# MikeIvanichev/norma

Measured on AMD Instinct MI355X. Metric: audio-sec/wall-sec (xRT) distil-large-v3 fp16 b32, higher is better.
Workload: dtype f16

## Files before the change

### norma_amd/csrc/k_attn_enc.hip

```cpp
#include "nh_kernels.h"

#ifndef ENC_ATTN_KERNEL
#define ENC_ATTN_KERNEL enc_attn_kernel
#define ENC_ATTN_LAUNCH launch_enc_attention
#endif
#define KT 64
#define QW 32
#ifndef ENC_ATTN_WAVES
#define ENC_ATTN_WAVES 8
#endif
#define QB (QW * ENC_ATTN_WAVES)
#define NTHR (64 * ENC_ATTN_WAVES)
#define NSLOT (NTHR >= 512 ? 1 : 512 / NTHR)
#define TILE_B 8192

__device__ __forceinline__ int swap23(int x) { return (x & ~12) | ((x & 4) << 1) | ((x & 8) >> 1); }

#ifndef ENC_ATTN_MINWAVES
#ifdef ENC_ATTN_PIPE
#define ENC_ATTN_MINWAVES 2
#else
#define ENC_ATTN_MINWAVES 4
#endif
#endif
__global__ __launch_bounds__(NTHR, (NTHR <= 512 ? ENC_ATTN_MINWAVES : 1)) void ENC_ATTN_KERNEL(const half_t *__restrict__ q, const half_t *__restrict__ k,
                                                         long ld, const half_t *__restrict__ vt,
                                                         half_t *__restrict__ out, long ldo, int S, int H) {
    __shared__ __attribute__((aligned(16))) char smem[2 * 2 * TILE_B];
    const int tid = threadIdx.x, lane = tid & 63, w = tid >> 6;
    const int r = lane & 31, hh = lane >> 5;
    const int b = blockIdx.z, h = blockIdx.y;
    const int q0 = blockIdx.x * QB + w * QW;
    const int nT = (S + KT - 1) / KT;

    half8 qf[4];
    {
        int qrow = q0 + r; if (qrow >= S) qrow = S - 1;
        const half_t *qp = q + ((long)b * S + qrow) * ld + h * NH_DH + 8 * hh;
#pragma unroll
        for (int ks = 0; ks < 4; ks++) qf[ks] = *reinterpret_cast<const half8 *>(qp + 16 * ks);
    }
    const half_t *kg[NSLOT]; const half_t *vg[NSLOT];
    int krow_off[NSLOT];
#pragma unroll
    for (int i = 0; i < NSLOT; i++) {
        int row = (tid >> 3) + (NTHR / 8) * i;
        int c = (tid & 7) ^ ((row >> 1) & 7);
        krow_off[i] = swap23(row);
        kg[i] = k + (long)b * S * ld + h * NH_DH + c * 8;
        vg[i] = vt + ((long)(b * H + h) * NH_DH + row) * NH_SP + c * 8;
    }
    u32x4 rk[NSLOT], rv[NSLOT];
    const bool stager = NTHR <= 512 || tid < 512;
    auto load_k = [&](int t) {
        if (!stager) return;
#pragma unroll
        for (int i = 0; i < NSLOT; i++) {
            int key = t * KT + krow_off[i]; if (key >= S) key = S - 1;
            rk[i] = *reinterpret_cast<const u32x4 *>(kg[i] + (long)key * ld);
        }
    };
    auto load_v = [&](int t) {
        if (!stager) return;
#pragma unroll
        for (int i = 0; i < NSLOT; i++) rv[i] = *reinterpret_cast<const u32x4 *>(vg[i] + t * KT);
    };
    auto store_k = [&](int buf) {
        if (!stager) return;
        u32x4 *lk = reinterpret_cast<u32x4 *>(smem + buf * 2 * TILE_B);
#pragma unroll
        for (int i = 0; i < NSLOT; i++) lk[tid + NTHR * i] = rk[i];
    };
    auto store_v = [&](int buf) {
        if (!stager) return;
        u32x4 *lv = reinterpret_cast<u32x4 *>(smem + buf * 2 * TILE_B + TILE_B);
#pragma unroll
        for (int i = 0; i < NSLOT; i++) lv[tid + NTHR * i] = rv[i];
    };
    auto load_tile = [&](int t) { load_k(t); load_v(t); };
    auto store_tile = [&](int buf) { store_k(buf); store_v(buf); };
    load_tile(0);
    store_tile(0);
#ifdef ENC_ATTN_PIPE
    if (nT > 1) { load_k(1); store_k(1); }
#endif
    __syncthreads();

    const int g = (r >> 1) & 7;
    const int offK0 = r * 128 + ((hh ^ g) << 4);
    const int offV0 = r * 128 + ((hh ^ g) << 4);

    f32x16 o0, o1;
#pragma unroll
    for (int i = 0; i < 16; i++) { o0[i] = 0.f; o1[i] = 0.f; }
    const f32x16 zero = {0.f, 0.f, 0.f, 0.f, 0.f, 0.f, 0.f, 0.f, 0.f, 0.f, 0.f, 0.f, 0.f, 0.f, 0.f, 0.f};
    const half_t one_h = hh == 0 ? (half_t)1.0f : (half_t)0.0f;
    const half8 kx = {one_h, one_h, (half_t)0.f, (half_t)0.f, (half_t)0.f, (half_t)0.f, (half_t)0.f, (half_t)0.f};
    half8 qx = {(half_t)0.f, (half_t)0.f, (half_t)0.f, (half_t)0.f, (half_t)0.f, (half_t)0.f, (half_t)0.f, (half_t)0.f};
    float m_ref = 0.f, l_run = 0.f;
    const float REBASE = 8.0f;

    f32x16 s0, s1;
    auto qk_phase = [&](const char *tk, f32x16 &s0, f32x16 &s1) {
        {
            half8 k0 = *reinterpret_cast<const half8 *>(tk + offK0);
            half8 k1 = *reinterpret_cast<const half8 *>(tk + 4096 + offK0);
            s0 = __builtin_amdgcn_mfma_f32_32x32x16_f16(k0, qf[0], zero, 0, 0, 0);
            s1 = __builtin_amdgcn_mfma_f32_32x32x16_f16(k1, qf[0], zero, 0, 0, 0);
        }
#pragma unroll
        for (int ks = 1; ks < 4; ks++) {
            half8 k0 = *reinterpret_cast<const half8 *>(tk + (offK0 ^ (ks << 5)));
            half8 k1 = *reinterpret_cast<const half8 *>(tk + 4096 + (offK0 ^ (ks << 5)));
            s0 = __builtin_amdgcn_mfma_f32_32x32x16_f16(k0, qf[ks], s0, 0, 0, 0);
            s1 = __builtin_amdgcn_mfma_f32_32x32x16_f16(k1, qf[ks], s1, 0, 0, 0);
        }
        s0 = __builtin_amdgcn_mfma_f32_32x32x16_f16(kx, qx, s0, 0, 0, 0);
        s1 = __builtin_amdgcn_mfma_f32_32x32x16_f16(kx, qx, s1, 0, 0, 0);
    };
    auto sm_head = [&](int t) {
        if (t * KT + KT > S) {
#pragma unroll
            for (int i = 0; i < 16; i++) {
                int rho = (i & 3) + 8 * (i >> 2) + 4 * hh;
                int key0 = t * KT + swap23(rho), key1 = t * KT + 32 + swap23(rho);
                if (key0 >= S) s0[i] = -INFINITY;
                if (key1 >= S) s1[i] = -INFINITY;
            }
        }
        float mx = fmaxf(fmaxf(s0[0], s0[1]), s0[2]);
#pragma unroll
        for (int i = 3; i < 15; i += 2) mx = fmaxf(fmaxf(mx, s0[i]), s0[i + 1]);
        mx = fmaxf(fmaxf(mx, s0[15]), s1[0]);
#pragma unroll
        for (int i = 1; i < 15; i += 2) mx = fmaxf(fmaxf(mx, s1[i]), s1[i + 1]);
        mx = fmaxf(mx, s1[15]);
        mx = fmaxf(mx, __shfl_xor(mx, 32));
        const bool reb = (t == 0) || (mx > REBASE);
        if (__builtin_amdgcn_ballot_w64(reb) != 0) {
            const float dlt = reb ? mx : 0.f;
            const float alpha = __builtin_amdgcn_exp2f(-dlt);
#pragma unroll
            for (int i = 0; i < 16; i++) { o0[i] *= alpha; o1[i] *= alpha; s0[i] -= dlt; s1[i] -= dlt; }
            l_run *= alpha;
            m_ref += dlt;
            const float nm = fminf(fmaxf(-m_ref, -60000.f), 60000.f);
            const half_t hi = (half_t)nm;
            const half_t lo = (half_t)(nm - (float)hi);
            qx[0] = hh == 0 ? hi : (half_t)0.f;
            qx[1] = hh == 0 ? lo : (half_t)0.f;
        }
    };
    auto sm_body = [&](const char *tv) {
        float ps = 0.f;
#pragma unroll
        for (int i = 0; i < 16; i++) {
            s0[i] = __builtin_amdgcn_exp2f(s0[i]); s1[i] = __builtin_amdgcn_exp2f(s1[i]);
            ps += s0[i]; ps += s1[i];
        }
        l_run += ps;
        half8 p00, p01, p10, p11;
#pragma unroll
        for (int j = 0; j < 8; j++) {
            p00[j] = (half_t)s0[j]; p01[j] = (half_t)s0[8 + j];
            p10[j] = (half_t)s1[j]; p11[j] = (half_t)s1[8 + j];
        }
        {
            half8 v;
            v = *reinterpret_cast<const half8 *>(tv + (offV0 ^ (0 << 4)));          o0 = __builtin_amdgcn_mfma_f32_32x32x16_f16(v, p00, o0, 0, 0, 0);
            v = *reinterpret_cast<const half8 *>(tv + 4096 + (offV0 ^ (0 << 4)));   o1 = __builtin_amdgcn_mfma_f32_32x32x16_f16(v, p00, o1, 0, 0, 0);
            v = *reinterpret_cast<const half8 *>(tv + (offV0 ^ (2 << 4)));          o0 = __builtin_amdgcn_mfma_f32_32x32x16_f16(v, p01, o0, 0, 0, 0);
            v = *reinterpret_cast<const half8 *>(tv + 4096 + (offV0 ^ (2 << 4)));   o1 = __builtin_amdgcn_mfma_f32_32x32x16_f16(v, p01, o1, 0, 0, 0);
            v = *reinterpret_cast<const half8 *>(tv + (offV0 ^ (4 << 4)));          o0 = __builtin_amdgcn_mfma_f32_32x32x16_f16(v, p10, o0, 0, 0, 0);
            v = *reinterpret_cast<const half8 *>(tv + 4096 + (offV0 ^ (4 << 4)));   o1 = __builtin_amdgcn_mfma_f32_32x32x16_f16(v, p10, o1, 0, 0, 0);
            v = *reinterpret_cast<const half8 *>(tv + (offV0 ^ (6 << 4)));          o0 = __builtin_amdgcn_mfma_f32_32x32x16_f16(v, p11, o0, 0, 0, 0);
            v = *reinterpret_cast<const half8 *>(tv + 4096 + (offV0 ^ (6 << 4)));   o1 = __builtin_amdgcn_mfma_f32_32x32x16_f16(v, p11, o1, 0, 0, 0);
        }
    };
#ifndef ENC_ATTN_PIPE
    int cur = 0;
    for (int t = 0; t < nT; t++) {
        const bool more = (t + 1 < nT);
        if (more) load_tile(t + 1);
        qk_phase(smem + cur * 2 * TILE_B, s0, s1);
        sm_head(t);
        sm_body(smem + cur * 2 * TILE_B + TILE_B);
        if (more) store_tile(cur ^ 1);
        __syncthreads();
        cur ^= 1;
    }
#else
    f32x16 n0, n1;
    qk_phase(smem, s0, s1);
    for (int t = 0; t < nT; t++) {
        if (t + 2 < nT) load_k(t + 2);
        if (t + 1 < nT) load_v(t + 1);
        sm_head(t);
        qk_phase(smem + ((t + 1) & 1) * 2 * TILE_B, n0, n1);
        sm_body(smem + (t & 1) * 2 * TILE_B + TILE_B);
#pragma unroll
        for (int i = 0; i < 18; i++) {
            __builtin_amdgcn_sched_group_barrier(0x008, 1, 0);
            __builtin_amdgcn_sched_group_barrier(0x002, ENC_ATTN_PIPE, 0);
        }
        if (t + 2 < nT) store_k(t & 1);
        if (t + 1 < nT) store_v((t + 1) & 1);
        __syncthreads();
        s0 = n0; s1 = n1;
    }
#endif
    const float l_tot = l_run + __shfl_xor(l_run, 32);
    const float inv = 1.0f / l_tot;
    const int qrow = q0 + r;
    if (qrow < S) {
        half_t *op = out + ((long)b * S + qrow) * ldo + h * NH_DH + 4 * hh;
#pragma unroll
        for (int gq = 0; gq < 4; gq++) {
            half4 a = {(half_t)(o0[4 * gq] * inv), (half_t)(o0[4 * gq + 1] * inv), (half_t)(o0[4 * gq + 2] * inv),
                       (half_t)(o0[4 * gq + 3] * inv)};
            half4 c = {(half_t)(o1[4 * gq] * inv), (half_t)(o1[4 * gq + 1] * inv), (half_t)(o1[4 * gq + 2] * inv),
                       (half_t)(o1[4 * gq + 3] * inv)};
            *reinterpret_cast<half4 *>(op + 8 * gq) = a;
            *reinterpret_cast<half4 *>(op + 32 + 8 * gq) = c;
        }
    }
}

void ENC_ATTN_LAUNCH(const half_t *q, const half_t *k, long ld, const half_t *vt, half_t *out, long ldo,
                          int B, int S, int H, hipStream_t st) {
    dim3 grid((S + QB - 1) / QB, H, B);
    hipLaunchKernelGGL(ENC_ATTN_KERNEL, grid, dim3(NTHR), 0, st, q, k, ld, vt, out, ldo, S, H);
}
```

### norma_amd/csrc/k_gemm.hip

```cpp
#include <stdlib.h>

#include <atomic>

#include "nh_kernels.h"

#define BM 128
#define BN 128
#define BK 64
#define TILE_BYTES (BM * BK * 2)

__device__ __forceinline__ float gelu_tanh_f(float v) { return gelu_tanh_fast(v); }

__device__ __forceinline__ const half_t *a_row_ptr(const GemmParams &p, int m) {
    if (m >= p.M) m = p.M - 1;
    int b = nh_div(m, p.a_rpb, p.a_magic), r = m - b * p.a_rpb;
    return p.A + (long)b * p.a_bstride + (long)r * p.lda;
}

typedef __attribute__((address_space(3))) void lds_void;
typedef const __attribute__((address_space(1))) void gbl_void;

template <bool SWAP>
__device__ __forceinline__ void gemm_mainloop(const GemmParams &p, char *smem, int m0, int n0,
                                              f32x4 (&acc)[4][4]) {
    const int tid = threadIdx.x, lane = tid & 63, w = tid >> 6;
    const int wm = w >> 1, wn = w & 1;
    const int cq = tid & 7;
    const half_t *ag[4], *wg[4];
#pragma unroll
    for (int i = 0; i < 4; i++) {
        int row = (tid >> 3) + 32 * i;
        int c = cq ^ ((row >> 1) & 7);
        ag[i] = a_row_ptr(p, m0 + row) + c * 8;
        int n = n0 + row;
        wg[i] = p.W + (long)n * p.K + c * 8;
    }
    const int nt = p.K / BK;
    const int fr = lane & 15, fq = lane >> 4;
    int offA[4], offB[4];
#pragma unroll
    for (int j = 0; j < 4; j++) {
        int rowA = wm * 64 + 16 * j + fr;
        int rowB = wn * 64 + 16 * j + fr;
        offA[j] = rowA * 128 + ((fq ^ ((rowA >> 1) & 7)) << 4);
        offB[j] = rowB * 128 + ((fq ^ ((rowB >> 1) & 7)) << 4);
    }
    const int wbase = __builtin_amdgcn_readfirstlane(w) * 1024;
    auto stage = [&](int buf, int t) {
        char *la = smem + buf * 2 * TILE_BYTES + wbase, *lb = la + TILE_BYTES;
#pragma unroll
        for (int i = 0; i < 4; i++) {
            __builtin_amdgcn_global_load_lds((gbl_void *)(ag[i] + (long)t * BK), (lds_void *)(la + 4096 * i), 16, 0, 0);
            __builtin_amdgcn_global_load_lds((gbl_void *)(wg[i] + (long)t * BK), (lds_void *)(lb + 4096 * i), 16, 0, 0);
        }
    };
    stage(0, 0);
    asm volatile("s_waitcnt vmcnt(0)" ::: "memory");
    __syncthreads();
    int cur = 0;
    for (int t = 0; t < nt; t++) {
        const bool more = (t + 1 < nt);
        if (more) stage(cur ^ 1, t + 1);
        const char *ta = smem + cur * 2 * TILE_BYTES, *tb = ta + TILE_BYTES;
#pragma unroll
        for (int ks = 0; ks < 2; ks++) {
            half8 fa[4], fb[4];
#pragma unroll
            for (int j = 0; j < 4; j++) {
                fa[j] = *reinterpret_cast<const half8 *>(ta + (offA[j] ^ (ks << 6)));
                fb[j] = *reinterpret_cast<const half8 *>(tb + (offB[j] ^ (ks << 6)));
            }
#pragma unroll
            for (int i = 0; i < 4; i++)
#pragma unroll
                for (int j = 0; j < 4; j++) {
                    if (SWAP)
                        acc[i][j] = __builtin_amdgcn_mfma_f32_16x16x32_f16(fb[i], fa[j], acc[i][j], 0, 0, 0);
                    else
                        acc[i][j] = __builtin_amdgcn_mfma_f32_16x16x32_f16(fa[j], fb[i], acc[i][j], 0, 0, 0);
                }
        }
        asm volatile("s_waitcnt vmcnt(0)" ::: "memory");
        __syncthreads();
        cur ^= 1;
    }
}

__device__ __forceinline__ long out_row(const GemmParams &p, int m) {
    int b = nh_div(m, p.o_rpb, p.o_magic), r = m - b * p.o_rpb;
    return (long)b * p.o_bstride + r + p.o_off;
}

__global__ __launch_bounds__(256, 2) void gemm_f16_kernel(GemmParams p) {
    __shared__ __attribute__((aligned(16))) char smem[4 * TILE_BYTES];
    const int ntn = p.N / BN, ntm = (p.M + BM - 1) / BM;
    const int nwg = ntn * ntm;
    int bid = blockIdx.x;
    {
        int xcd = bid & 7, q = nwg >> 3, r = nwg & 7;
        bid = (xcd < r ? xcd * (q + 1) : r * (q + 1) + (xcd - r) * q) + (bid >> 3);
    }
    const int tm = bid / ntn, tn = bid - tm * ntn;
    const int m0 = tm * BM, n0 = tn * BN;
    const int lane = threadIdx.x & 63, w = threadIdx.x >> 6;
    const int wm = w >> 1, wn = w & 1;
    const int fr = lane & 15, fq = lane >> 4;

    f32x4 acc[4][4];
#pragma unroll
    for (int i = 0; i < 4; i++)
#pragma unroll
        for (int j = 0; j < 4; j++) acc[i][j] = (f32x4){0.f, 0.f, 0.f, 0.f};

    const int seg = (p.epi == EPI_F16 || p.epi == EPI_GELU_F16) ? n0 / p.seg_n : 0;
    const bool vt = (p.epi == EPI_F16 && seg == p.vt_seg);
    if (vt) gemm_mainloop<false>(p, smem, m0, n0, acc);
    else gemm_mainloop<true>(p, smem, m0, n0, acc);

    if (vt) {
        half_t *dst = reinterpret_cast<half_t *>(seg == 0 ? p.out[0] : seg == 1 ? p.out[1] : p.out[2]);
#pragma unroll
        for (int i = 0; i < 4; i++) {
            int n = n0 + wn * 64 + 16 * i + fr;
            float bv = p.bias ? p.bias[n] : 0.f;
            int nl = n - seg * p.seg_n, h = nl >> 6, dh = nl & 63;
#pragma unroll
            for (int j = 0; j < 4; j++) {
                int m = m0 + wm * 64 + 16 * j + 4 * fq;
                if (m >= p.M) continue;
                int b = nh_div(m, p.S, p.s_magic), s = m - b * p.S;
                half_t *row = dst + ((long)(b * p.H + h) * NH_DH + dh) * NH_SP;
                if (s + 3 < p.S && m + 3 < p.M) {
                    half4 v = {(half_t)(acc[i][j][0] + bv), (half_t)(acc[i][j][1] + bv),
                               (half_t)(acc[i][j][2] + bv), (half_t)(acc[i][j][3] + bv)};
                    *reinterpret_cast<half4 *>(row + s) = v;
                } else {
                    for (int r = 0; r < 4; r++) {
                        int mm = m + r;
                        if (mm >= p.M) break;
                        int bb = nh_div(mm, p.S, p.s_magic), ss = mm - bb * p.S;
                        dst[((long)(bb * p.H + h) * NH_DH + dh) * NH_SP + ss] = (half_t)(acc[i][j][r] + bv);
                    }
                }
            }
        }
        return;
    }
    half_t *obase = reinterpret_cast<half_t *>(seg == 0 ? p.out[0] : seg == 1 ? p.out[1] : p.out[2]);
#pragma unroll
    for (int i = 0; i < 4; i++) {
        const int n = n0 + wn * 64 + 16 * i + 4 * fq;
        f32x4 bv = {0.f, 0.f, 0.f, 0.f};
        if (p.bias) bv = *reinterpret_cast<const f32x4 *>(p.bias + n);
#pragma unroll
        for (int j = 0; j < 4; j++) {
            const int m = m0 + wm * 64 + 16 * j + fr;
            if (m >= p.M) continue;
            f32x4 v = acc[i][j] + bv;
            if (p.epi == EPI_F16 || p.epi == EPI_GELU_F16) {
                if (p.epi == EPI_F16 && seg == 0 && p.seg0_scale != 0.f) v *= p.seg0_scale;
                if (p.epi == EPI_GELU_F16) {
                    v[0] = gelu_tanh_f(v[0]); v[1] = gelu_tanh_f(v[1]);
                    v[2] = gelu_tanh_f(v[2]); v[3] = gelu_tanh_f(v[3]);
                }
                const int nl = n - seg * p.seg_n;
                half_t *dst = p.head_major ? obase + (((long)nh_div(m, p.S, p.s_magic) * p.H + (nl >> 6)) * p.S + (m - nh_div(m, p.S, p.s_magic) * p.S)) * NH_DH + (nl & 63)
                                           : obase + out_row(p, m) * p.ldo + nl;
                half4 hv = {(half_t)v[0], (half_t)v[1], (half_t)v[2], (half_t)v[3]};
                *reinterpret_cast<half4 *>(dst) = hv;
            } else if (p.epi == EPI_RESID_F32) {
                float *dst = reinterpret_cast<float *>(p.out[0]) + (long)m * p.ldo + n;
                f32x4 x = *reinterpret_cast<const f32x4 *>(dst);
                *reinterpret_cast<f32x4 *>(dst) = x + v;
            } else {
                int s = m - nh_div(m, p.S, p.s_magic) * p.S;
                f32x4 pe = *reinterpret_cast<const f32x4 *>(p.pos + (long)s * p.N + n);
                f32x4 o = {gelu_tanh_f(v[0]) + pe[0], gelu_tanh_f(v[1]) + pe[1], gelu_tanh_f(v[2]) + pe[2],
                           gelu_tanh_f(v[3]) + pe[3]};
                *reinterpret_cast<f32x4 *>(reinterpret_cast<float *>(p.out[0]) + (long)m * p.ldo + n) = o;
            }
        }
    }
}

#define G2_BM 256
#define G2_BN 256
#ifndef G2_GM
#define G2_GM 4
#endif
#define PP_BUF 65536
#define PP_HT 16384
#define PP_RING (2 * PP_BUF)
#define PP_EPI_PITCH 136
#define PP_EPI_WAVE (16 * PP_EPI_PITCH)

struct PPSource { unsigned ag[2][2], wg[2][2]; };

__device__ __forceinline__ PPSource pp_source(const GemmParams &p, int m0, int n0) {
    int tid = threadIdx.x;
    asm volatile("" : "+v"(tid));
    const int lrow = tid >> 3;
    const int csrc = ((tid & 7) ^ ((lrow >> 1) & 7)) * 8;
    PPSource sg;
#pragma unroll
    for (int h = 0; h < 2; h++)
#pragma unroll
        for (int i = 0; i < 2; i++) {
            sg.ag[h][i] = (unsigned)(a_row_ptr(p, m0 + i * 128 + h * 64 + lrow) - p.A) + csrc;
            const int l = lrow + 64 * i;
            sg.wg[h][i] = (unsigned)(n0 + (l >> 5) * 64 + h * 32 + (l & 31)) * (unsigned)p.K + csrc;
        }
    return sg;
}

__device__ __forceinline__ void pp_stage(const GemmParams &p, char *wbase, const PPSource &sg, int t, int which) {
    const int h = (which >> 1) & 1;
    const bool isB = which == 1 || which == 2;
    char *dst = wbase + (t & 1) * PP_BUF + (isB ? 2 * PP_HT : 0) + h * PP_HT;
    const unsigned ko = (unsigned)t * 64u;
    if (isB) {
        __builtin_amdgcn_global_load_lds((gbl_void *)(p.W + (size_t)(sg.wg[h][0] + ko)), (lds_void *)dst, 16, 0, 0);
        __builtin_amdgcn_global_load_lds((gbl_void *)(p.W + (size_t)(sg.wg[h][1] + ko)), (lds_void *)(dst + 8192), 16, 0, 0);
    } else {
        __builtin_amdgcn_global_load_lds((gbl_void *)(p.A + (size_t)(sg.ag[h][0] + ko)), (lds_void *)dst, 16, 0, 0);
        __builtin_amdgcn_global_load_lds((gbl_void *)(p.A + (size_t)(sg.ag[h][1] + ko)), (lds_void *)(dst + 8192), 16, 0, 0);
    }
}

__device__ __forceinline__ void pp_prologue(const GemmParams &p, char *wbase, const PPSource &sg) {
    pp_stage(p, wbase, sg, 0, 0); pp_stage(p, wbase, sg, 0, 1); pp_stage(p, wbase, sg, 0, 2); pp_stage(p, wbase, sg, 0, 3);
    pp_stage(p, wbase, sg, 1, 0); pp_stage(p, wbase, sg, 1, 1);
}

template <bool SWAP>
__device__ __forceinline__ void pp_main(const GemmParams &p, char *smem, char *wbase, const PPSource &sg, f32x4 (&acc)[8][4]) {
    const int lane = threadIdx.x & 63, w = threadIdx.x >> 6;
    const int wr = w >> 2, wc = w & 3;
    const int fr = lane & 15, fq = lane >> 4;
    const int nt = p.K >> 6;
    const int offA0 = (wr * 64 + fr) * 128 + ((fq ^ (fr >> 1)) << 4);
    const int offB0 = (wc * 32 + fr) * 128 + ((fq ^ (fr >> 1)) << 4);
    const char *const pa[2] = {smem + offA0, smem + (offA0 ^ 64)};
    const char *const pb[2] = {smem + offB0, smem + (offB0 ^ 64)};
    half8 fa[4][2], fb[4][2];

#define PP_PHASE(Q, BUF, WAIT, DO_ISSUE, ST)                                                                             \
    {                                                                                                                    \
        constexpr int tb_ = (BUF) * PP_BUF;                                                                              \
        if ((Q) == 0) {                                                                                                  \
            _Pragma("unroll") for (int j = 0; j < 2; j++) _Pragma("unroll") for (int ks = 0; ks < 2; ks++)             \
                fb[j][ks] = *reinterpret_cast<const half8 *>(pb[ks] + (tb_ + 2 * PP_HT + 2048 * j));                    \
            __builtin_amdgcn_sched_barrier(0);                                                                           \
            _Pragma("unroll") for (int i = 0; i < 4; i++) _Pragma("unroll") for (int ks = 0; ks < 2; ks++)             \
                fa[i][ks] = *reinterpret_cast<const half8 *>(pa[ks] + (tb_ + 2048 * i));                               \
        } else if ((Q) == 1) {                                                                                           \
            _Pragma("unroll") for (int j = 0; j < 2; j++) _Pragma("unroll") for (int ks = 0; ks < 2; ks++)             \
                fb[2 + j][ks] = *reinterpret_cast<const half8 *>(pb[ks] + (tb_ + 3 * PP_HT + 2048 * j));                \
        } else if ((Q) == 2) {                                                                                           \
            _Pragma("unroll") for (int i = 0; i < 4; i++) _Pragma("unroll") for (int ks = 0; ks < 2; ks++)             \
                fa[i][ks] = *reinterpret_cast<const half8 *>(pa[ks] + (tb_ + PP_HT + 2048 * i));                       \
        }                                                                                                                \
        __builtin_amdgcn_sched_barrier(0);                                                                               \
        if (DO_ISSUE) pp_stage(p, wbase, sg, (ST), (Q) == 2 ? 0 : (Q) == 3 ? 1 : (Q) == 0 ? 2 : 3);                     \
        if ((WAIT) == 8) asm volatile("s_waitcnt vmcnt(8)" ::: "memory");                                                \
        else if ((WAIT) == 4) asm volatile("s_waitcnt vmcnt(4)" ::: "memory");                                           \
        else if ((WAIT) == 2) asm volatile("s_waitcnt vmcnt(2)" ::: "memory");                                           \
        else if ((WAIT) == 0) asm volatile("s_waitcnt vmcnt(0)" ::: "memory");                                           \
        __builtin_amdgcn_s_barrier();                                                                                    \
        asm volatile("s_waitcnt lgkmcnt(0)" ::: "memory");                                                               \
        __builtin_amdgcn_sched_barrier(0);                                                                               \
        __builtin_amdgcn_s_setprio(1);                                                                                   \
        {                                                                                                                \
            constexpr int ib_ = ((Q) >= 2) ? 4 : 0, jb_ = ((Q) == 1 || (Q) == 2) ? 2 : 0;                                \
            _Pragma("unroll") for (int ks = 0; ks < 2; ks++) _Pragma("unroll") for (int i = 0; i < 4; i++)             \
                _Pragma("unroll") for (int j = 0; j < 2; j++) {                                                         \
                    if (SWAP) acc[ib_ + i][jb_ + j] = __builtin_amdgcn_mfma_f32_16x16x32_f16(fb[jb_ + j][ks], fa[i][ks], acc[ib_ + i][jb_ + j], 0, 0, 0); \
                    else acc[ib_ + i][jb_ + j] = __builtin_amdgcn_mfma_f32_16x16x32_f16(fa[i][ks], fb[jb_ + j][ks], acc[ib_ + i][jb_ + j], 0, 0, 0);      \
                }                                                                                                        \
        }                                                                                                                \
        __builtin_amdgcn_s_setprio(0);                                                                                   \
        __builtin_amdgcn_sched_barrier(0);                                                                               \
        __builtin_amdgcn_s_barrier();                                                                                    \
    }

    asm volatile("s_waitcnt vmcnt(0)" ::: "memory");
    __builtin_amdgcn_s_barrier();
    if (wr == 1) __builtin_amdgcn_s_barrier();
    int t = 0;
    for (; t + 4 <= nt; t += 2) {
        PP_PHASE(0, 0, 8, true, t + 1)
        PP_PHASE(1, 0, 8, true, t + 1)
        PP_PHASE(2, 0, -1, true, t + 2)
        PP_PHASE(3, 0, 8, true, t + 2)
        PP_PHASE(0, 1, 8, true, t + 2)
        PP_PHASE(1, 1, 8, true, t + 2)
        PP_PHASE(2, 1, -1, true, t + 3)
        PP_PHASE(3, 1, 8, true, t + 3)
    }
    PP_PHASE(0, 0, 8, true, t + 1)
    PP_PHASE(1, 0, 8, true, t + 1)
    PP_PHASE(2, 0, -1, false, 0)
    PP_PHASE(3, 0, 4, false, 0)
    PP_PHASE(0, 1, 2, false, 0)
    PP_PHASE(1, 1, 0, false, 0)
    PP_PHASE(2, 1, -1, false, 0)
    PP_PHASE(3, 1, -1, false, 0)
    if (wr == 0) __builtin_amdgcn_s_barrier();
#undef PP_PHASE
}

__device__ __forceinline__ void pp_tile(int vb, int ntn, int ntm, int &tm, int &tn) {
    const int nwg = ntn * ntm;
    const int xcd = vb & 7, q = nwg >> 3, r = nwg & 7;
    const int bid = (xcd < r ? xcd * (q + 1) : r * (q + 1) + (xcd - r) * q) + (vb >> 3);
    const int per_group = G2_GM * ntn;
    const int g = bid / per_group, rr = bid - g * per_group;
    const int gm = min(G2_GM, ntm - g * G2_GM);
    tn = rr / gm; tm = g * G2_GM + (rr - tn * gm);
}

template <int EPI>
__global__ __launch_bounds__(512) void gemm256_f16_kernel(GemmParams p) {
    __shared__ __attribute__((aligned(16))) char smem[PP_RING + 8 * PP_EPI_WAVE];
    const int ntn = p.N / G2_BN, ntm = (p.M + G2_BM - 1) / G2_BM, nwg = ntn * ntm;
    const int lane = threadIdx.x & 63, w = threadIdx.x >> 6;
    const int wm = w >> 2, wn = w & 3;
    const int fr = lane & 15, fq = lane >> 4;
    char *const wbase = smem + __builtin_amdgcn_readfirstlane(w) * 1024;
    char *const img = smem + PP_RING + w * PP_EPI_WAVE;

    int vb = blockIdx.x, tm, tn;
    pp_tile(vb, ntn, ntm, tm, tn);
    PPSource sg = pp_source(p, tm * G2_BM, tn * G2_BN);
    pp_prologue(p, wbase, sg);
#ifdef G2_STAMPS
    int stamp_n = 0;
    if (threadIdx.x == 0 && p.dbg) {
        p.dbg[blockIdx.x * 32 + 0] = __builtin_amdgcn_s_memrealtime();
        p.dbg[blockIdx.x * 32 + 1] = __builtin_amdgcn_s_getreg(6164);
    }
#endif
    for (;;) {
        const int m0 = tm * G2_BM, n0 = tn * G2_BN;
        f32x4 acc[8][4];
#pragma unroll
        for (int i = 0; i < 8; i++)
#pragma unroll
            for (int j = 0; j < 4; j++) acc[i][j] = (f32x4){0.f, 0.f, 0.f, 0.f};
        const int seg = (EPI == EPI_F16 || EPI == EPI_GELU_F16) ? n0 / p.seg_n : 0;
        const bool vt = (EPI == EPI_F16 && seg == p.vt_seg);
        if (vt) pp_main<false>(p, smem, wbase, sg, acc);
        else pp_main<true>(p, smem, wbase, sg, acc);

#ifdef G2_STAMPS
        if (threadIdx.x == 0 && p.dbg) p.dbg[blockIdx.x * 32 + 3] += __builtin_amdgcn_s_memrealtime() - (stamp_n ? p.dbg[blockIdx.x * 32 + 4 + stamp_n - 1] : p.dbg[blockIdx.x * 32]);
#endif
        f32x4 rs[4][4];
        __amdgpu_buffer_rsrc_t xrs;
        unsigned xoff = 0;
        if (EPI == EPI_RESID_F32) {
            xrs = __builtin_amdgcn_make_buffer_rsrc(p.out[0], 0, (int)((long)p.M * p.ldo * 4), 0x00020000);
            int ln = threadIdx.x;
            asm volatile("" : "+v"(ln));
            xoff = (unsigned)(((long)(m0 + (ln >> 8) * 128 + (ln & 15)) * p.ldo + n0 + ((ln >> 6) & 3) * 64 + 4 * ((ln >> 4) & 3)) * 4);
#pragma unroll
            for (int ii = 0; ii < 4; ii++)
#pragma unroll
                for (int j = 0; j < 4; j++)
                    rs[ii][j] = __builtin_bit_cast(f32x4, __builtin_amdgcn_raw_buffer_load_b128(xrs, xoff + (unsigned)(64 * ii * p.ldo + 64 * j), 0, 0));
        }
        const int nvb = vb + gridDim.x;
        const bool more = nvb < nwg;
        if (more) {
            pp_tile(nvb, ntn, ntm, tm, tn);
            sg = pp_source(p, tm * G2_BM, tn * G2_BN);
            pp_prologue(p, wbase, sg);
        }

        if (vt) {
            half_t *dst = reinterpret_cast<half_t *>(seg == 0 ? p.out[0] : seg == 1 ? p.out[1] : p.out[2]);
#pragma unroll
            for (int j = 0; j < 4; j++) {
                const float bv = p.bias ? p.bias[n0 + wn * 64 + 16 * j + fr] : 0.f;
#pragma unroll
                for (int hh = 0; hh < 2; hh++) {
#pragma unroll
                    for (int ii = 0; ii < 4; ii++) {
                        const f32x4 a = acc[4 * hh + ii][j];
                        half4 v = {(half_t)(a[0] + bv), (half_t)(a[1] + bv), (half_t)(a[2] + bv), (half_t)(a[3] + bv)};
                        *reinterpret_cast<half4 *>(img + fr * PP_EPI_PITCH + (16 * ii + 4 * fq) * 2) = v;
                    }
#pragma unroll
                    for (int it = 0; it < 2; it++) {
                        const int nrow = 8 * it + (lane >> 3), mc = (lane & 7) * 8;
                        const half4 lo = *reinterpret_cast<const half4 *>(img + nrow * PP_EPI_PITCH + mc * 2);
                        const half4 hi = *reinterpret_cast<const half4 *>(img + nrow * PP_EPI_PITCH + mc * 2 + 8);
                        const int n = n0 + wn * 64 + 16 * j + nrow, nl = n - seg * p.seg_n, h = nl >> 6, dh = nl & 63;
                        const int m = m0 + wm * 128 + 64 * hh + mc;
                        if (m >= p.M) continue;
                        const int b = nh_div(m, p.S, p.s_magic), ss = m - b * p.S;
                        if (ss + 7 < p.S && m + 7 < p.M) {
                            half8 o = {lo[0], lo[1], lo[2], lo[3], hi[0], hi[1], hi[2], hi[3]};
                            *reinterpret_cast<half8 *>(dst + ((long)(b * p.H + h) * NH_DH + dh) * NH_SP + ss) = o;
                        } else {
                            for (int r = 0; r < 8; r++) {
                                const int mm = m + r;
                                if (mm >= p.M) break;
                                const int bb = nh_div(mm, p.S, p.s_magic), s2 = mm - bb * p.S;
                                dst[((long)(bb * p.H + h) * NH_DH + dh) * NH_SP + s2] = r < 4 ? lo[r] : hi[r - 4];
                            }
                        }
                    }
                }
            }
        } else if (EPI == EPI_F16 || EPI == EPI_GELU_F16) {
            half_t *ob = reinterpret_cast<half_t *>(seg == 0 ? p.out[0] : seg == 1 ? p.out[1] : p.out[2]);
            f32x4 bv[4];
#pragma unroll
            for (int j = 0; j < 4; j++) {
                bv[j] = (f32x4){0.f, 0.f, 0.f, 0.f};
                if (p.bias) bv[j] = *reinterpret_cast<const f32x4 *>(p.bias + n0 + wn * 64 + 16 * j + 4 * fq);
            }
            const int ncol = n0 + wn * 64 - seg * p.seg_n + (lane & 7) * 8;
            const bool q_scaled = EPI == EPI_F16 && seg == 0 && p.seg0_scale != 0.f;
#pragma unroll
            for (int i = 0; i < 8; i++) {
#pragma unroll
                for (int j = 0; j < 4; j++) {
                    f32x4 v = acc[i][j] + bv[j];
                    if (EPI == EPI_F16 && q_scaled) v *= p.seg0_scale;
                    if (EPI == EPI_GELU_F16) {
                        v[0] = gelu_tanh_f(v[0]); v[1] = gelu_tanh_f(v[1]); v[2] = gelu_tanh_f(v[2]); v[3] = gelu_tanh_f(v[3]);
                    }
                    half4 hv = {(half_t)v[0], (half_t)v[1], (half_t)v[2], (half_t)v[3]};
                    *reinterpret_cast<half4 *>(img + fr * PP_EPI_PITCH + (16 * j + 4 * fq) * 2) = hv;
                }
#pragma unroll
                for (int it = 0; it < 2; it++) {
                    const int mr = 8 * it + (lane >> 3);
                    const int m = m0 + wm * 128 + 16 * i + mr;
                    const half4 lo = *reinterpret_cast<const half4 *>(img + mr * PP_EPI_PITCH + (lane & 7) * 16);
                    const half4 hi = *reinterpret_cast<const half4 *>(img + mr * PP_EPI_PITCH + (lane & 7) * 16 + 8);
                    if (m < p.M) {
                        half8 o = {lo[0], lo[1], lo[2], lo[3], hi[0], hi[1], hi[2], hi[3]};
                        half_t *dst = p.head_major ? ob + (((long)nh_div(m, p.S, p.s_magic) * p.H + (ncol >> 6)) * p.S + (m - nh_div(m, p.S, p.s_magic) * p.S)) * NH_DH + (lane & 7) * 8
                                                   : ob + out_row(p, m) * p.ldo + ncol;
                        *reinterpret_cast<half8 *>(dst) = o;
                    }
                }
            }
        } else if (EPI == EPI_RESID_F32) {
            f32x4 bv[4];
#pragma unroll
            for (int j = 0; j < 4; j++) {
                bv[j] = (f32x4){0.f, 0.f, 0.f, 0.f};
                if (p.bias) bv[j] = *reinterpret_cast<const f32x4 *>(p.bias + n0 + wn * 64 + 16 * j + 4 * fq);
            }
#pragma unroll
            for (int ii = 0; ii < 4; ii++)
#pragma unroll
                for (int j = 0; j < 4; j++)
                    __builtin_amdgcn_raw_buffer_store_b128(__builtin_bit_cast(u32x4, rs[ii][j] + (acc[ii][j] + bv[j])), xrs, xoff + (unsigned)(64 * ii * p.ldo + 64 * j), 0, 0);
#pragma unroll
            for (int ii = 0; ii < 4; ii++)
#pragma unroll
                for (int j = 0; j < 4; j++)
                    rs[ii][j] = __builtin_bit_cast(f32x4, __builtin_amdgcn_raw_buffer_load_b128(xrs, xoff + (unsigned)(64 * (4 + ii) * p.ldo + 64 * j), 0, 0));
#pragma unroll
            for (int ii = 0; ii < 4; ii++)
#pragma unroll
                for (int j = 0; j < 4; j++)
                    __builtin_amdgcn_raw_buffer_store_b128(__builtin_bit_cast(u32x4, rs[ii][j] + (acc[4 + ii][j] + bv[j])), xrs, xoff + (unsigned)(64 * (4 + ii) * p.ldo + 64 * j), 0, 0);
        } else {
#pragma unroll
            for (int j = 0; j < 4; j++) {
                const int n = n0 + wn * 64 + 16 * j + 4 * fq;
                f32x4 bv = {0.f, 0.f, 0.f, 0.f};
                if (p.bias) bv = *reinterpret_cast<const f32x4 *>(p.bias + n);
#pragma unroll
                for (int i = 0; i < 8; i++) {
                    const int m = m0 + wm * 128 + 16 * i + fr;
                    if (m >= p.M) continue;
                    const f32x4 v = acc[i][j] + bv;
                    const int s = m - nh_div(m, p.S, p.s_magic) * p.S;
                    const f32x4 pe = *reinterpret_cast<const f32x4 *>(p.pos + (long)s * p.N + n);
                    f32x4 o = {gelu_tanh_f(v[0]) + pe[0], gelu_tanh_f(v[1]) + pe[1], gelu_tanh_f(v[2]) + pe[2],
                               gelu_tanh_f(v[3]) + pe[3]};
                    *reinterpret_cast<f32x4 *>(reinterpret_cast<float *>(p.out[0]) + (long)m * p.ldo + n) = o;
                }
            }
        }
        if (!more) break;
        vb = nvb;
    }
}

static int device_cu_count() {
    static std::atomic<int> cus[NH_MAX_DEVICES];
    int dev = 0;
    if (hipGetDevice(&dev) != hipSuccess || dev < 0 || dev >= NH_MAX_DEVICES) return 256;
    int n = cus[dev].load(std::memory_order_relaxed);
    if (!n) {
        if (hipDeviceGetAttribute(&n, hipDeviceAttributeMultiprocessorCount, dev) != hipSuccess || n <= 0) n = 256;
        cus[dev].store(n, std::memory_order_relaxed);
    }
    return n;
}

static GemmParams with_magics(const GemmParams &p_in) {
    GemmParams p = p_in;
    const long max_m = (long)p.M - 1;
    p.a_magic = nh_magic(p.a_rpb, max_m); p.o_magic = nh_magic(p.o_rpb, max_m); p.s_magic = nh_magic(p.S, max_m);
    return p;
}

void launch_gemm(const GemmParams &p_in, hipStream_t st) {
    const GemmParams p = with_magics(p_in);
    const bool seg_ok = (p.epi != EPI_F16 && p.epi != EPI_GELU_F16) || (p.seg_n % G2_BN == 0);
    if (p.N % G2_BN == 0 && p.K % 128 == 0 && seg_ok && p.M >= G2_BM) {
        const int nwg = (p.N / G2_BN) * ((p.M + G2_BM - 1) / G2_BM);
        int cus = p.cus > 0 ? p.cus : device_cu_count();
        cus -= cus % 8;
        const dim3 grid(nwg < cus ? nwg : cus), block(512);
        switch (p.epi) {
            case EPI_F16: hipLaunchKernelGGL(gemm256_f16_kernel<EPI_F16>, grid, block, 0, st, p); break;
            case EPI_GELU_F16: hipLaunchKernelGGL(gemm256_f16_kernel<EPI_GELU_F16>, grid, block, 0, st, p); break;
            case EPI_RESID_F32: hipLaunchKernelGGL(gemm256_f16_kernel<EPI_RESID_F32>, grid, block, 0, st, p); break;
            default: hipLaunchKernelGGL(gemm256_f16_kernel<EPI_CONV2_F32>, grid, block, 0, st, p); break;
        }
        return;
    }
    launch_gemm_128(p, st);
}

void launch_gemm_128(const GemmParams &p_in, hipStream_t st) {
    const GemmParams p = with_magics(p_in);
    int ntn = p.N / BN, ntm = (p.M + BM - 1) / BM;
    hipLaunchKernelGGL(gemm_f16_kernel, dim3(ntn * ntm), dim3(256), 0, st, p);
}
```

Measured before the change: 6901.

## Stage bias in LDS, inline-asm residual prefetch, and trim register pressure in GEMM epilogue

The 256-tile GEMM now stages each tile's bias into LDS before the mainloop and reads it from LDS in the epilogue. The residual prefetch is rewritten as inline buffer_load asm with partial vmcnt waits. Thread and lane index math is deferred and rematerialized via asm barriers and readfirstlane so fewer values stay live across the mainloop. A g_div helper replaces nh_div with a magic-number or runtime-divide choice, and the encoder attention recomputes its output row indices late, using ds_bpermute for the final reduction, to shorten live ranges. The extra LDS for bias and the hand-written waitcnt add occupancy and correctness risk.

```diff
diff --git a/norma_amd/csrc/k_attn_enc.hip b/norma_amd/csrc/k_attn_enc.hip
--- a/norma_amd/csrc/k_attn_enc.hip
+++ b/norma_amd/csrc/k_attn_enc.hip
@@ -85,6 +85,7 @@
     if (nT > 1) { load_k(1); store_k(1); }
 #endif
     __syncthreads();
+    asm volatile("" : "+v"(qf[0]), "+v"(qf[1]), "+v"(qf[2]), "+v"(qf[3]) :: "memory");
 
     const int g = (r >> 1) & 7;
     const int offK0 = r * 128 + ((hh ^ g) << 4);
@@ -209,11 +210,13 @@
         s0 = n0; s1 = n1;
     }
 #endif
-    const float l_tot = l_run + __shfl_xor(l_run, 32);
+    int te = threadIdx.x;
+    asm volatile("" : "+v"(te));
+    const float l_tot = l_run + __builtin_bit_cast(float, __builtin_amdgcn_ds_bpermute(((te ^ 32) & 63) << 2, __builtin_bit_cast(int, l_run)));
     const float inv = 1.0f / l_tot;
-    const int qrow = q0 + r;
+    const int qrow = blockIdx.x * QB + (te >> 6) * QW + (te & 31);
     if (qrow < S) {
-        half_t *op = out + ((long)b * S + qrow) * ldo + h * NH_DH + 4 * hh;
+        half_t *op = out + ((long)b * S + qrow) * ldo + h * NH_DH + 4 * ((te >> 5) & 1);
 #pragma unroll
         for (int gq = 0; gq < 4; gq++) {
             half4 a = {(half_t)(o0[4 * gq] * inv), (half_t)(o0[4 * gq + 1] * inv), (half_t)(o0[4 * gq + 2] * inv),
diff --git a/norma_amd/csrc/k_gemm.hip b/norma_amd/csrc/k_gemm.hip
--- a/norma_amd/csrc/k_gemm.hip
+++ b/norma_amd/csrc/k_gemm.hip
@@ -11,9 +11,18 @@
 
 __device__ __forceinline__ float gelu_tanh_f(float v) { return gelu_tanh_fast(v); }
 
+__device__ __forceinline__ int g_div(int m, int d, unsigned magic) {
+    if (magic == 0u) return 0;
+    if (magic == ~0u) {
+        asm volatile("" : "+s"(d));
+        return m / d;
+    }
+    return (int)__umulhi((unsigned)m, magic);
+}
+
 __device__ __forceinline__ const half_t *a_row_ptr(const GemmParams &p, int m) {
     if (m >= p.M) m = p.M - 1;
-    int b = nh_div(m, p.a_rpb, p.a_magic), r = m - b * p.a_rpb;
+    int b = g_div(m, p.a_rpb, p.a_magic), r = m - b * p.a_rpb;
     return p.A + (long)b * p.a_bstride + (long)r * p.lda;
 }
 
@@ -87,7 +96,7 @@
 }
 
 __device__ __forceinline__ long out_row(const GemmParams &p, int m) {
-    int b = nh_div(m, p.o_rpb, p.o_magic), r = m - b * p.o_rpb;
+    int b = g_div(m, p.o_rpb, p.o_magic), r = m - b * p.o_rpb;
     return (long)b * p.o_bstride + r + p.o_off;
 }
 
@@ -128,7 +137,7 @@
             for (int j = 0; j < 4; j++) {
                 int m = m0 + wm * 64 + 16 * j + 4 * fq;
                 if (m >= p.M) continue;
-                int b = nh_div(m, p.S, p.s_magic), s = m - b * p.S;
+                int b = g_div(m, p.S, p.s_magic), s = m - b * p.S;
                 half_t *row = dst + ((long)(b * p.H + h) * NH_DH + dh) * NH_SP;
                 if (s + 3 < p.S && m + 3 < p.M) {
                     half4 v = {(half_t)(acc[i][j][0] + bv), (half_t)(acc[i][j][1] + bv),
@@ -138,7 +147,7 @@
                     for (int r = 0; r < 4; r++) {
                         int mm = m + r;
                         if (mm >= p.M) break;
-                        int bb = nh_div(mm, p.S, p.s_magic), ss = mm - bb * p.S;
+                        int bb = g_div(mm, p.S, p.s_magic), ss = mm - bb * p.S;
                         dst[((long)(bb * p.H + h) * NH_DH + dh) * NH_SP + ss] = (half_t)(acc[i][j][r] + bv);
                     }
                 }
@@ -164,7 +173,7 @@
                     v[2] = gelu_tanh_f(v[2]); v[3] = gelu_tanh_f(v[3]);
                 }
                 const int nl = n - seg * p.seg_n;
-                half_t *dst = p.head_major ? obase + (((long)nh_div(m, p.S, p.s_magic) * p.H + (nl >> 6)) * p.S + (m - nh_div(m, p.S, p.s_magic) * p.S)) * NH_DH + (nl & 63)
+                half_t *dst = p.head_major ? obase + (((long)g_div(m, p.S, p.s_magic) * p.H + (nl >> 6)) * p.S + (m - g_div(m, p.S, p.s_magic) * p.S)) * NH_DH + (nl & 63)
                                            : obase + out_row(p, m) * p.ldo + nl;
                 half4 hv = {(half_t)v[0], (half_t)v[1], (half_t)v[2], (half_t)v[3]};
                 *reinterpret_cast<half4 *>(dst) = hv;
@@ -173,7 +182,7 @@
                 f32x4 x = *reinterpret_cast<const f32x4 *>(dst);
                 *reinterpret_cast<f32x4 *>(dst) = x + v;
             } else {
-                int s = m - nh_div(m, p.S, p.s_magic) * p.S;
+                int s = m - g_div(m, p.S, p.s_magic) * p.S;
                 f32x4 pe = *reinterpret_cast<const f32x4 *>(p.pos + (long)s * p.N + n);
                 f32x4 o = {gelu_tanh_f(v[0]) + pe[0], gelu_tanh_f(v[1]) + pe[1], gelu_tanh_f(v[2]) + pe[2],
                            gelu_tanh_f(v[3]) + pe[3]};
@@ -193,6 +202,7 @@
 #define PP_RING (2 * PP_BUF)
 #define PP_EPI_PITCH 136
 #define PP_EPI_WAVE (16 * PP_EPI_PITCH)
+#define PP_BIAS (512 * 4)
 
 struct PPSource { unsigned ag[2][2], wg[2][2]; };
 
@@ -234,31 +244,38 @@
 
 template <bool SWAP>
 __device__ __forceinline__ void pp_main(const GemmParams &p, char *smem, char *wbase, const PPSource &sg, f32x4 (&acc)[8][4]) {
-    const int lane = threadIdx.x & 63, w = threadIdx.x >> 6;
+    int tid = threadIdx.x;
+    asm volatile("" : "+v"(tid));
+    const int lane = tid & 63, w = __builtin_amdgcn_readfirstlane(tid >> 6);
     const int wr = w >> 2, wc = w & 3;
     const int fr = lane & 15, fq = lane >> 4;
     const int nt = p.K >> 6;
     const int offA0 = (wr * 64 + fr) * 128 + ((fq ^ (fr >> 1)) << 4);
     const int offB0 = (wc * 32 + fr) * 128 + ((fq ^ (fr >> 1)) << 4);
-    const char *const pa[2] = {smem + offA0, smem + (offA0 ^ 64)};
-    const char *const pb[2] = {smem + offB0, smem + (offB0 ^ 64)};
+    int oa[2][2] = {{offA0, offA0 ^ 64}, {offA0 + PP_BUF, (offA0 ^ 64) + PP_BUF}};
+    int ob[2][2] = {{offB0, offB0 ^ 64}, {offB0 + PP_BUF, (offB0 ^ 64) + PP_BUF}};
+#pragma unroll
+    for (int b = 0; b < 2; b++)
+#pragma unroll
+        for (int ks = 0; ks < 2; ks++) asm volatile("" : "+v"(oa[b][ks]), "+v"(ob[b][ks]));
+    const char *const pa[2][2] = {{smem + oa[0][0], smem + oa[0][1]}, {smem + oa[1][0], smem + oa[1][1]}};
+    const char *const pb[2][2] = {{smem + ob[0][0], smem + ob[0][1]}, {smem + ob[1][0], smem + ob[1][1]}};
     half8 fa[4][2], fb[4][2];
 
 #define PP_PHASE(Q, BUF, WAIT, DO_ISSUE, ST)                                                                             \
     {                                                                                                                    \
-        constexpr int tb_ = (BUF) * PP_BUF;                                                                              \
         if ((Q) == 0) {                                                                                                  \
             _Pragma("unroll") for (int j = 0; j < 2; j++) _Pragma("unroll") for (int ks = 0; ks < 2; ks++)             \
-                fb[j][ks] = *reinterpret_cast<const half8 *>(pb[ks] + (tb_ + 2 * PP_HT + 2048 * j));                    \
+                fb[j][ks] = *reinterpret_cast<const half8 *>(pb[BUF][ks] + (2 * PP_HT + 2048 * j));                    \
             __builtin_amdgcn_sched_barrier(0);                                                                           \
             _Pragma("unroll") for (int i = 0; i < 4; i++) _Pragma("unroll") for (int ks = 0; ks < 2; ks++)             \
-                fa[i][ks] = *reinterpret_cast<const half8 *>(pa[ks] + (tb_ + 2048 * i));                               \
+                fa[i][ks] = *reinterpret_cast<const half8 *>(pa[BUF][ks] + 2048 * i);                               \
         } else if ((Q) == 1) {                                                                                           \
             _Pragma("unroll") for (int j = 0; j < 2; j++) _Pragma("unroll") for (int ks = 0; ks < 2; ks++)             \
-                fb[2 + j][ks] = *reinterpret_cast<const half8 *>(pb[ks] + (tb_ + 3 * PP_HT + 2048 * j));                \
+                fb[2 + j][ks] = *reinterpret_cast<const half8 *>(pb[BUF][ks] + (3 * PP_HT + 2048 * j));                \
         } else if ((Q) == 2) {                                                                                           \
             _Pragma("unroll") for (int i = 0; i < 4; i++) _Pragma("unroll") for (int ks = 0; ks < 2; ks++)             \
-                fa[i][ks] = *reinterpret_cast<const half8 *>(pa[ks] + (tb_ + PP_HT + 2048 * i));                       \
+                fa[i][ks] = *reinterpret_cast<const half8 *>(pa[BUF][ks] + (PP_HT + 2048 * i));                       \
         }                                                                                                                \
         __builtin_amdgcn_sched_barrier(0);                                                                               \
         if (DO_ISSUE) pp_stage(p, wbase, sg, (ST), (Q) == 2 ? 0 : (Q) == 3 ? 1 : (Q) == 0 ? 2 : 3);                     \
@@ -321,13 +338,9 @@
 
 template <int EPI>
 __global__ __launch_bounds__(512) void gemm256_f16_kernel(GemmParams p) {
-    __shared__ __attribute__((aligned(16))) char smem[PP_RING + 8 * PP_EPI_WAVE];
+    __shared__ __attribute__((aligned(16))) char smem[PP_RING + 8 * PP_EPI_WAVE + PP_BIAS];
     const int ntn = p.N / G2_BN, ntm = (p.M + G2_BM - 1) / G2_BM, nwg = ntn * ntm;
-    const int lane = threadIdx.x & 63, w = threadIdx.x >> 6;
-    const int wm = w >> 2, wn = w & 3;
-    const int fr = lane & 15, fq = lane >> 4;
-    char *const wbase = smem + __builtin_amdgcn_readfirstlane(w) * 1024;
-    char *const img = smem + PP_RING + w * PP_EPI_WAVE;
+    char *const wbase = smem + __builtin_amdgcn_readfirstlane(threadIdx.x >> 6) * 1024;
 
     int vb = blockIdx.x, tm, tn;
     pp_tile(vb, ntn, ntm, tm, tn);
@@ -349,25 +362,41 @@
             for (int j = 0; j < 4; j++) acc[i][j] = (f32x4){0.f, 0.f, 0.f, 0.f};
         const int seg = (EPI == EPI_F16 || EPI == EPI_GELU_F16) ? n0 / p.seg_n : 0;
         const bool vt = (EPI == EPI_F16 && seg == p.vt_seg);
+        if (EPI != EPI_CONV2_F32) {
+            int tb = threadIdx.x;
+            asm volatile("" : "+v"(tb));
+            reinterpret_cast<float *>(smem + PP_RING + 8 * PP_EPI_WAVE)[tb] = p.bias ? p.bias[n0 + (tb & 255)] : 0.f;
+        }
         if (vt) pp_main<false>(p, smem, wbase, sg, acc);
         else pp_main<true>(p, smem, wbase, sg, acc);
 
 #ifdef G2_STAMPS
-        if (threadIdx.x == 0 && p.dbg) p.dbg[blockIdx.x * 32 + 3] += __builtin_amdgcn_s_memrealtime() - (stamp_n ? p.dbg[blockIdx.x * 32 + 4 + stamp_n - 1] : p.dbg[blockIdx.x * 32]);
+        if (threadIdx.x == 0 && p.dbg && stamp_n < 28) p.dbg[blockIdx.x * 32 + 3] += __builtin_amdgcn_s_memrealtime() - (stamp_n ? p.dbg[blockIdx.x * 32 + 4 + stamp_n - 1] : p.dbg[blockIdx.x * 32]);
 #endif
+        int ln = threadIdx.x;
+        asm volatile("" : "+v"(ln));
+        const int lane = ln & 63, w = __builtin_amdgcn_readfirstlane(ln >> 6);
+        const int wm = w >> 2, wn = w & 3;
+        const int fr = lane & 15, fq = lane >> 4;
+        char *const img = smem + PP_RING + w * PP_EPI_WAVE;
+        const float *const bst = reinterpret_cast<const float *>(smem + PP_RING + 8 * PP_EPI_WAVE) + w * 64;
         f32x4 rs[4][4];
         __amdgpu_buffer_rsrc_t xrs;
         unsigned xoff = 0;
         if (EPI == EPI_RESID_F32) {
             xrs = __builtin_amdgcn_make_buffer_rsrc(p.out[0], 0, (int)((long)p.M * p.ldo * 4), 0x00020000);
-            int ln = threadIdx.x;
-            asm volatile("" : "+v"(ln));
-            xoff = (unsigned)(((long)(m0 + (ln >> 8) * 128 + (ln & 15)) * p.ldo + n0 + ((ln >> 6) & 3) * 64 + 4 * ((ln >> 4) & 3)) * 4);
-#pragma unroll
-            for (int ii = 0; ii < 4; ii++)
-#pragma unroll
-                for (int j = 0; j < 4; j++)
-                    rs[ii][j] = __builtin_bit_cast(f32x4, __builtin_amdgcn_raw_buffer_load_b128(xrs, xoff + (unsigned)(64 * ii * p.ldo + 64 * j), 0, 0));
+            const unsigned long long xa = reinterpret_cast<unsigned long long>(p.out[0]);
+            const u32x4 xrw = {(unsigned)xa, (unsigned)(xa >> 32) & 0xffffu, (unsigned)((long)p.M * p.ldo * 4), 0x00020000u};
+            xoff =(unsigned)(((long)(m0 + (ln >> 8) * 128 + (ln & 15)) * p.ldo + n0 + ((ln >> 6) & 3) * 64 + 4 * ((ln >> 4) & 3)) * 4);
+#pragma unroll
+            for (int ii = 0; ii < 4; ii++) {
+                const unsigned vo = xoff + (unsigned)(64 * ii * p.ldo);
+                asm volatile("buffer_load_dwordx4 %0, %4, %5, 0 offen\n\t"
+                             "buffer_load_dwordx4 %1, %4, %5, 0 offen offset:64\n\t"
+                             "buffer_load_dwordx4 %2, %4, %5, 0 offen offset:128\n\t"
+                             "buffer_load_dwordx4 %3, %4, %5, 0 offen offset:192"
+                             : "=&v"(rs[ii][0]), "=&v"(rs[ii][1]), "=&v"(rs[ii][2]), "=&v"(rs[ii][3]) : "v"(vo), "s"(xrw) : "memory");
+            }
         }
         const int nvb = vb + gridDim.x;
         const bool more = nvb < nwg;
@@ -376,12 +405,17 @@
             sg = pp_source(p, tm * G2_BM, tn * G2_BN);
             pp_prologue(p, wbase, sg);
         }
+        if (EPI == EPI_RESID_F32) {
+            if (!more) asm volatile("s_waitcnt vmcnt(0)" ::: "memory");
+            asm volatile("s_waitcnt vmcnt(12)" : "+v"(rs[0][0]), "+v"(rs[0][1]), "+v"(rs[0][2]), "+v"(rs[0][3]), "+v"(rs[1][0]), "+v"(rs[1][1]), "+v"(rs[1][2]), "+v"(rs[1][3]) :: "memory");
+            asm volatile("" : "+v"(rs[2][0]), "+v"(rs[2][1]), "+v"(rs[2][2]), "+v"(rs[2][3]), "+v"(rs[3][0]), "+v"(rs[3][1]), "+v"(rs[3][2]), "+v"(rs[3][3]) :: "memory");
+        }
 
         if (vt) {
             half_t *dst = reinterpret_cast<half_t *>(seg == 0 ? p.out[0] : seg == 1 ? p.out[1] : p.out[2]);
 #pragma unroll
             for (int j = 0; j < 4; j++) {
-                const float bv = p.bias ? p.bias[n0 + wn * 64 + 16 * j + fr] : 0.f;
+                const float bv = bst[16 * j + fr];
 #pragma unroll
                 for (int hh = 0; hh < 2; hh++) {
 #pragma unroll
@@ -398,7 +432,7 @@
                         const int n = n0 + wn * 64 + 16 * j + nrow, nl = n - seg * p.seg_n, h = nl >> 6, dh = nl & 63;
                         const int m = m0 + wm * 128 + 64 * hh + mc;
                         if (m >= p.M) continue;
-                        const int b = nh_div(m, p.S, p.s_magic), ss = m - b * p.S;
+                        const int b = g_div(m, p.S, p.s_magic), ss = m - b * p.S;
                         if (ss + 7 < p.S && m + 7 < p.M) {
                             half8 o = {lo[0], lo[1], lo[2], lo[3], hi[0], hi[1], hi[2], hi[3]};
                             *reinterpret_cast<half8 *>(dst + ((long)(b * p.H + h) * NH_DH + dh) * NH_SP + ss) = o;
@@ -406,7 +440,7 @@
                             for (int r = 0; r < 8; r++) {
                                 const int mm = m + r;
                                 if (mm >= p.M) break;
-                                const int bb = nh_div(mm, p.S, p.s_magic), s2 = mm - bb * p.S;
+                                const int bb = g_div(mm, p.S, p.s_magic), s2 = mm - bb * p.S;
                                 dst[((long)(bb * p.H + h) * NH_DH + dh) * NH_SP + s2] = r < 4 ? lo[r] : hi[r - 4];
                             }
                         }
@@ -417,10 +451,7 @@
             half_t *ob = reinterpret_cast<half_t *>(seg == 0 ? p.out[0] : seg == 1 ? p.out[1] : p.out[2]);
             f32x4 bv[4];
 #pragma unroll
-            for (int j = 0; j < 4; j++) {
-                bv[j] = (f32x4){0.f, 0.f, 0.f, 0.f};
-                if (p.bias) bv[j] = *reinterpret_cast<const f32x4 *>(p.bias + n0 + wn * 64 + 16 * j + 4 * fq);
-            }
+            for (int j = 0; j < 4; j++) bv[j] = *reinterpret_cast<const f32x4 *>(bst + 16 * j + 4 * fq);
             const int ncol = n0 + wn * 64 - seg * p.seg_n + (lane & 7) * 8;
             const bool q_scaled = EPI == EPI_F16 && seg == 0 && p.seg0_scale != 0.f;
 #pragma unroll
@@ -443,7 +474,7 @@
                     const half4 hi = *reinterpret_cast<const half4 *>(img + mr * PP_EPI_PITCH + (lane & 7) * 16 + 8);
                     if (m < p.M) {
                         half8 o = {lo[0], lo[1], lo[2], lo[3], hi[0], hi[1], hi[2], hi[3]};
-                        half_t *dst = p.head_major ? ob + (((long)nh_div(m, p.S, p.s_magic) * p.H + (ncol >> 6)) * p.S + (m - nh_div(m, p.S, p.s_magic) * p.S)) * NH_DH + (lane & 7) * 8
+                        half_t *dst = p.head_major ? ob + (((long)g_div(m, p.S, p.s_magic) * p.H + (ncol >> 6)) * p.S + (m - g_div(m, p.S, p.s_magic) * p.S)) * NH_DH + (lane & 7) * 8
                                                    : ob + out_row(p, m) * p.ldo + ncol;
                         *reinterpret_cast<half8 *>(dst) = o;
                     }
@@ -452,10 +483,7 @@
         } else if (EPI == EPI_RESID_F32) {
             f32x4 bv[4];
 #pragma unroll
-            for (int j = 0; j < 4; j++) {
-                bv[j] = (f32x4){0.f, 0.f, 0.f, 0.f};
-                if (p.bias) bv[j] = *reinterpret_cast<const f32x4 *>(p.bias + n0 + wn * 64 + 16 * j + 4 * fq);
-            }
+            for (int j = 0; j < 4; j++) bv[j] = *reinterpret_cast<const f32x4 *>(bst + 16 * j + 4 * fq);
 #pragma unroll
             for (int ii = 0; ii < 4; ii++)
 #pragma unroll
@@ -482,7 +510,7 @@
                     const int m = m0 + wm * 128 + 16 * i + fr;
                     if (m >= p.M) continue;
                     const f32x4 v = acc[i][j] + bv;
-                    const int s = m - nh_div(m, p.S, p.s_magic) * p.S;
+                    const int s = m - g_div(m, p.S, p.s_magic) * p.S;
                     const f32x4 pe = *reinterpret_cast<const f32x4 *>(p.pos + (long)s * p.N + n);
                     f32x4 o = {gelu_tanh_f(v[0]) + pe[0], gelu_tanh_f(v[1]) + pe[1], gelu_tanh_f(v[2]) + pe[2],
                                gelu_tanh_f(v[3]) + pe[3]};
@@ -490,6 +518,9 @@
                 }
             }
         }
+#ifdef G2_STAMPS
+        if (threadIdx.x == 0 && p.dbg && stamp_n < 28) { p.dbg[blockIdx.x * 32 + 4 + stamp_n] = __builtin_amdgcn_s_memrealtime(); stamp_n++; p.dbg[blockIdx.x * 32 + 2] = stamp_n; }
+#endif
         if (!more) break;
         vb = nvb;
     }
```

Measured after the change: 6966, median of 6. About the same (+0.9%).
